# IllyaArtemchuk/Harmonies-Alphazero

Hardware: AMD Instinct MI355X
Metric: self-play env-steps/sec + games/sec @4096 boards, 1/2/4/8 GPUs; bit-exact vs CPU (higher is better)
Workload: dtype u64; 1 GPU; config2: 4096 concurrent boards/GPU, reset + rule-driven play to game end (legal mask, step, chance draws, final scoring); one step = 256 hz_play launches of 4096 boards; boards_per_gpu=4096, parallelism=shard1

## Files before the change

### harmonies-alphazero_amd/csrc/hz_env.hip

```cpp
#include <hip/hip_runtime.h>

#include <cstdio>
#include <cstdlib>
#include <cstring>

#include "../../include/hz_abi.h"
#include "hz_device.hpp"
#include "hz_encode.hpp"
#include "hz_host.hpp"

using namespace hz;
using namespace hz_host;

struct P2Draw {
  int32_t *tag;
  int32_t *k;
  uint64_t *q;
  uint64_t *bag;
  int32_t *c;
};
struct P2Mid {
  int32_t *tag;
  uint64_t *st;
  uint64_t *q;
  int32_t *i;
};

#ifndef HZ_P2_NDRAW
#define HZ_P2_NDRAW 6
#endif
#ifndef HZ_P2_NPLAY
#define HZ_P2_NPLAY 5
#endif
constexpr int kP2Draw = HZ_P2_NDRAW;
constexpr int kP2Play = HZ_P2_NPLAY;
constexpr int kP2SDraw = 4;
constexpr int kP2SPlay = kP2SDraw + kP2Draw;
constexpr int kP2Stages = kP2SPlay + kP2Play;
constexpr int kP2Last = kP2Stages - 1;
constexpr int kP2Ring = kP2Play + 1;
constexpr int kP2Stream = kP2Stages;
static_assert(kP2Draw >= 2 && kP2Draw <= 6 && kP2Play >= 2 && kP2Play <= 5, "stage counts");

struct hz_env {
  DevBufs bufs, p2_bufs, ar_bufs;
  int32_t n;
  uint64_t seed_base;
  hipStream_t stream;
  uint64_t *state;
  uint32_t *mt;
  int32_t *pos;
  int32_t *ply;
  int32_t *episode;
  uint64_t *seed;
  int seed_ahead;
  uint32_t *ahead_mt[2];
  int32_t *ahead_tag[2];
  uint64_t *ahead_pile[2];
  int32_t *ahead_cur[2];
  uint32_t *ahead_rule[2];
  int32_t *ep_final[2];
  size_t nrow;
  uint32_t *ring_mt[3];
  int32_t *ring_tag[3];
  uint64_t *ring_pile[3];
  int32_t *ring_cur[3];
  int32_t *ring_k1[3];
  int calls;
  int primed, slot_valid[2];
  int32_t *mt_src;
  int lazy;
  int ar_ahead;
  uint32_t *ar_mt;
  int32_t *ar_tag;
  uint64_t *ar_pile;
// ... 568 lines not shown
  a.seed_h[2] = e->p2_p3h[w];
  const int draws = e->seed_ahead;
  for (int k = 0; k < kP2Draw; k++) {
    P2DrawArgs &d = a.dr[k];
    const int s = kP2SDraw + k;
    d.slot = e->p2_s[sl(s)];
    d.stag = e->p2_s_tag[sl(s)];
    d.cur = e->p2_s_cur[sl(s)];
    d.in = e->p2_x[k > 0 ? k - 1 : 0][w];
    d.out = k == kP2Draw - 1 ? e->p2_pl[c % kP2Ring] : e->p2_x[k][r];
    d.d0 = e->p2_dcut[k];
    d.d1 = k == kP2Draw - 1 ? draws : std::min(draws, e->p2_dcut[k + 1]);
  }
  for (int st = 0; st < kP2Play; st++) {
    P2PlayArgs &p = a.pp[st];
    const bool last = st == kP2Play - 1;
    const int s = kP2SPlay + st;
    const int k = (c + kP2Ring - 1 - st) % kP2Ring;
    p.ep = last ? e->episode : e->p2_ep[w];
    p.ep_off = last ? 0 : kP2Play - 1 - st;
    p.g0 = st > 0 ? e->p2_cut[st - 1] : 0;
    p.g_end = last ? max_plies : std::min(e->p2_cut[st], max_plies);
    p.fell_lim = e->p2_fell_lim;
    p.ptag = e->p2_pl[k].tag;
    p.pk = e->p2_pl[k].k;
    p.q = st > 0 ? e->p2_m[st - 1][w].q : e->p2_pl[k].q;
    p.h = e->p2_h[sl(s)];
    p.slot = e->p2_s[sl(s)];
    p.cur = e->p2_s_cur[sl(s)];
    p.in = e->p2_m[st > 0 ? st - 1 : 0][w];
    p.out = e->p2_m[last ? 0 : st][r];
  }
  const int nblk = grid_for(e->n);
  hipLaunchKernelGGL(k_play2, dim3(4 * nblk), dim3(kStageThreads), kResetLds, e->stream, a, nblk);
  if (int err = launch_err()) return err;
  e->lazy = 1;
  e->calls2 = (c + 1) % (kP2Stream * kP2Ring * 2);
  e->primed = 0;
  e->ar_primed = 0;
  return 0;
}

extern "C" {

hz_env *hz_env_create(int32_t n_boards, uint64_t seed_base, void *stream) {
  if (n_boards <= 0) return nullptr;
  if (install_comp_table()) return nullptr;
  if (lds_opt_in<k_reset>(kResetLds) || lds_opt_in<k_rollout<false, false>>(kResetLds) ||
      lds_opt_in<k_rollout<false, true>>(kResetLds) || lds_opt_in<k_rollout<true, false>>(kResetLds) ||
      lds_opt_in<k_rollout<true, true>>(kResetLds) || lds_opt_in<k_play2>(kResetLds) ||
      lds_opt_in<k_mt_materialize2>(kResetLds))
    return nullptr;
  hz_env *e = new (std::nothrow) hz_env();
  if (!e) return nullptr;
  e->n = n_boards;
  e->seed_base = seed_base;
  e->stream = (hipStream_t)stream;
  const size_t n = (size_t)n_boards, nr = (n + kBlock - 1) / kBlock * kBlock, i32 = sizeof(int32_t);
  e->nrow = nr;
  DevBufs &o = e->bufs;
  o.get(e->state, n * 6 * sizeof(uint64_t), 0);
  o.get(e->mt, n * 624 * sizeof(uint32_t));
  o.get(e->pos, n * i32, 0);
  o.get(e->ply, n * i32, 0);
  o.get(e->episode, n * i32, 0);
  o.get(e->seed, n * sizeof(uint64_t), 0);
  o.get(e->mt_src, n * i32, 0xff);
// ... 325 lines not shown
  if (touch(e)) return 1;
  if (int err = materialize(e)) return err;
  hipLaunchKernelGGL(k_turn_op, dim3(grid_for(e->n)), dim3(kBlock), 0, e->stream, e->state, e->mt, e->pos, e->n, sel,
                     0);
  return launch_err();
}

int hz_end_turn(hz_env *e, const uint8_t *sel) {
  if (!e) return -1;
  if (touch(e)) return 1;
  if (int err = materialize(e)) return err;
  hipLaunchKernelGGL(k_turn_op, dim3(grid_for(e->n)), dim3(kBlock), 0, e->stream, e->state, e->mt, e->pos, e->n, sel,
                     1);
  return launch_err();
}

int hz_encode_states(const uint64_t *states, int64_t word_stride, int64_t item_stride, const int32_t *idx, int32_t m,
                     float *board, float *glob, void *stream) {
  if (!states || m < 0 || (!board && !glob)) return -1;
  if (m == 0) return 0;
  launch_encode(states, (long)word_stride, (long)item_stride, idx, m, board, glob, (hipStream_t)stream);
  return launch_err();
}

const char *hz_version(void) { return "hz 0.1 gfx950"; }

#ifdef HZ_DIAG
int hz_diag_set_stamps(uint64_t *p) {
  return hipMemcpyToSymbol(HIP_SYMBOL(g_stamps), &p, sizeof(p)) == hipSuccess ? 0 : 1;
}
int hz_diag_set_role_only(int r) {
  return hipMemcpyToSymbol(HIP_SYMBOL(g_role_only), &r, sizeof(r)) == hipSuccess ? 0 : 1;
}
#endif

}
```

### harmonies-alphazero_amd/csrc/hz_host.hpp

```cpp
#pragma once

#include <atomic>
#include <cstddef>
#include <cstdint>
#include <cstdio>
#include <cstdlib>
#include <new>
#include <vector>

namespace hz_host {

inline int env_int(const char *name, int dflt) {
  const char *e = getenv(name);
  return e ? atoi(e) : dflt;
}

inline int env_pick(const char *name, int special, int otherwise) {
  return env_int(name, otherwise) == special ? special : otherwise;
}

inline int env_clamped(const char *name, int dflt, int lo, int hi) {
  const int v = env_int(name, dflt);
  return v < lo ? lo : v > hi ? hi : v;
}
// ... 3 lines not shown
  int c[3];
  if (e && sscanf(e, "%d,%d,%d", &c[0], &c[1], &c[2]) == 3 && c[0] > 0 && c[1] > c[0] && c[2] > c[1] &&
      c[0] % 4 == 0 && c[1] % 4 == 0 && c[2] % 4 == 0)
    for (int k = 0; k < 3; k++) cut[k] = c[k];
}

inline bool env_cuts_n(const char *name, int *cut, int n, int step, int hi) {
  const char *e = getenv(name);
  if (!e || n < 1 || n > 8 || step < 1) return false;
  int c[8];
  for (int k = 0; k < n; k++) {
    if (*e < '0' || *e > '9') return false;
    long v = 0;
    for (; *e >= '0' && *e <= '9'; e++)
      if ((v = v * 10 + (*e - '0')) > hi) return false;
    if (v < step || v % step || (k && v <= c[k - 1])) return false;
    c[k] = (int)v;
    if (*e++ != (k + 1 < n ? ',' : '\0')) return false;
  }
  for (int k = 0; k < n; k++) cut[k] = c[k];
  return true;
}

inline bool cuts_gaps_within(const int *cut, int n, int max_gap) {
  for (int k = 0; k + 1 < n; k++)
    if (cut[k + 1] - cut[k] > max_gap) return false;
  return true;
}

inline bool env_p2_dcuts(const char *name, int *dcut, int ndraw, int draws, int max_gap) {
  if (ndraw < 2 || ndraw > 8) return false;
  int dc[9];
  for (int k = 0; k <= ndraw; k++) dc[k] = dcut[k];
  bool got = ndraw == 6 && env_cuts_n(name, dc + 1, 5, 1, draws);
  if (!got) {
    const int n = ndraw == 6 ? 4 : ndraw - 1;
    got = env_cuts_n(name, dc + 1, n, 1, draws - 1);
    if (got && ndraw == 6 && dc[5] < dc[4]) dc[5] = dc[4];
  }
  if (!got || !cuts_gaps_within(dc, ndraw + 1, max_gap)) return false;
  for (int k = 0; k <= ndraw; k++) dcut[k] = dc[k];
  return true;
}

struct Setting {
  static constexpr int64_t kUnread = INT64_MIN;
  const char *name;
  int32_t dflt;
  std::atomic<int64_t> v{kUnread};
  int32_t get() {
    int64_t x = v.load(std::memory_order_relaxed);
    if (x == kUnread) {
      int64_t expect = kUnread;
      v.compare_exchange_strong(expect, (int64_t)env_int(name, dflt));
      x = v.load(std::memory_order_relaxed);
    }
    return (int32_t)x;
  }
  void set(int32_t x) { v.store(x, std::memory_order_relaxed); }
};

template <class Dev>
struct DevBufsT {
  struct Held {
    void *p;
    void *slot;
    void (*clear)(void *slot);
  };
  std::vector<Held> held;
  bool ok = true;

// ... 71 lines not shown
```

### harmonies-alphazero_amd/csrc/hz_play2.hpp

```cpp
#pragma once

namespace {

#ifndef HZ_P2_ST_WT
#define HZ_P2_ST_WT 0
#endif
#ifndef HZ_P2_AUX
#define HZ_P2_AUX 16
#endif
#ifndef HZ_P2_STATIC_WIN
#define HZ_P2_STATIC_WIN 1
#endif
constexpr bool kP2StaticWin = HZ_P2_STATIC_WIN;

constexpr int kP2Win = 96;
constexpr int kP2WinRows = kP2Win + 24;
#ifndef HZ_P2_DCUT
#if HZ_P2_NDRAW == 6
#define HZ_P2_DCUT 0, 5, 9, 13, 17, 20
#elif HZ_P2_NDRAW == 5
#define HZ_P2_DCUT 0, 6, 11, 15, 19
#elif HZ_P2_NDRAW == 4
#define HZ_P2_DCUT 0, 7, 13, 18
#endif
#endif
constexpr int kP2DCut[kP2Draw] = {HZ_P2_DCUT};
constexpr int kP2StageDraws = 7;
#ifndef HZ_P2_PCUT
#if HZ_P2_NPLAY == 5
#define HZ_P2_PCUT 16, 32, 48, 64
#elif HZ_P2_NPLAY == 4
#define HZ_P2_PCUT 24, 40, 56
#endif
#endif
constexpr int kP2PCut[kP2Play - 1] = {HZ_P2_PCUT};
enum { kWvP1 = 8, kWvPlay = 10, kWvIdle = 15 };
#ifndef HZ_P2_WAVES
#if HZ_P2_NDRAW == 6 && HZ_P2_NPLAY == 5
#define HZ_P2_WAVES 0, 1, 4, 5, 2, 3, 8, 10
#elif HZ_P2_NDRAW == 6
#define HZ_P2_WAVES 0, 1, 4, 5, 2, 3, 8, 15
#elif HZ_P2_NDRAW == 5 && HZ_P2_NPLAY == 5
#define HZ_P2_WAVES 0, 1, 4, 15, 2, 3, 8, 10
#elif HZ_P2_NDRAW == 5
#define HZ_P2_WAVES 0, 1, 4, 15, 2, 3, 8, 15
#elif HZ_P2_NPLAY == 5
#define HZ_P2_WAVES 0, 1, 8, 15, 2, 3, 10, 15
#else
#define HZ_P2_WAVES 0, 1, 8, 15, 2, 3, 15, 15
#endif
#endif
constexpr int kP2Wave[8] = {HZ_P2_WAVES};
constexpr int p2_wave_count(int code) {
  int c = 0;
  for (int k = 0; k < 8; k++) c += kP2Wave[k] == code;
  return c;
}
constexpr bool p2_waves_ok() {
  for (int d = 0; d < 6; d++)
    if (p2_wave_count(d) != (d < kP2Draw ? 1 : 0)) return false;
  return p2_wave_count(kWvP1) == 1 && p2_wave_count(kWvPlay) == (kP2Play == 5 ? 1 : 0);
}
#ifndef HZ_P2_HSPLIT
#define HZ_P2_HSPLIT 24, 24, 52
#endif
constexpr int kP2HashSplit[3] = {HZ_P2_HSPLIT};
constexpr int kP2HashCut[5] = {0, kP2HashSplit[0], kP2HashSplit[1], kP2HashSplit[2], kRulePlies};
static_assert(0 <= kP2HashCut[1] && kP2HashCut[1] <= kP2HashCut[2] && kP2HashCut[2] <= kP2HashCut[3] &&
                  kP2HashCut[3] <= kRulePlies,
              "HZ_P2_HSPLIT: non-decreasing rows within the table");
static_assert(p2_waves_ok(), "HZ_P2_WAVES: every stage outside the seed and play blocks on exactly one wave");
constexpr int kP2MinPlies = 96;
#ifdef HZ_DIAG
constexpr int kP2Stamps = 48;
#define P2_PHASE(slot, t0)                                                                                       \
  do {                                                                                                           \
    __builtin_amdgcn_sched_barrier(0);                                                                           \
    if (g_stamps && b < a.n) g_stamps[(size_t)b * kP2Stamps + (slot)] = __builtin_amdgcn_s_memtime() - (t0); \
    __builtin_amdgcn_sched_barrier(0);                                                                           \
  } while (0)
#define P2_USE_V(x) asm volatile("" ::"v"(x))
#define P2_USE_S(x) asm volatile("" ::"s"(x))
#else
#define P2_PHASE(slot, t0) \
  do {                     \
  } while (0)
#define P2_USE_V(x) \
  do {              \
  } while (0)
#define P2_USE_S(x) \
  do {              \
  } while (0)
#endif
static_assert(4 * kP2WinRows * kWinStride * 4 <= (int)kResetLds, "a window per wave of a draw block");

struct P2DrawArgs {
  const uint32_t *slot;
  const int32_t *stag;
  int32_t *cur;
  P2Draw in, out;
  int d0, d1;
};
struct P2PlayArgs {
  const int32_t *ep;
  int ep_off;
  int g0;
  int g_end;
  int fell_lim;
  const int32_t *ptag, *pk;
  const uint64_t *q;
  const uint32_t *h;
  uint32_t *slot;
  const int32_t *cur;
  P2Mid in, out;
};
struct P2Args {
  uint64_t *st;
  uint32_t *mt;
  int32_t *pos, *ply, *episode;
  uint64_t *seed;
  int n, max_plies;
  uint64_t seed_base;
  long nrow;
  int32_t *games_done, *steps_done, *mt_src;
  int32_t *win_tag;
  const int32_t *ep_in;
  int32_t *ep_out;
  P2DrawArgs dr[kP2Draw];
  P2PlayArgs pp[kP2Play];
  uint32_t *s_mt[kP2SDraw];
  int32_t *s_tag[kP2SDraw];
  const int32_t *seed_tag[3];
  const uint32_t *seed_h[3];
  int s_idx_last;
  uint32_t *p1h_w;
  int32_t *p1t_w;
  uint32_t *p2h_w;
  uint32_t *p3h_w;
  uint32_t *s_h[kP2SDraw];
  int32_t *err;
  int spin;
};

struct PlayDraw2 : PileScript {
  bool fell;
  MTR gm;
  const int32_t *cur_nd;
  __device__ __forceinline__ bool pair_pops() const { return d + 2 <= nd; }
  __device__ __forceinline__ bool lost() const { return fell && gm.over(); }
  __device__ __forceinline__ uint32_t draw_one(uint64_t misc) {
    if (d < nd) return pop();
    if (!fell) {
      gm = MTR(gm.w, gm.stride, *cur_nd, gm.lim);
      fell = true;
    }
    uint32_t p9;
    return draw_pile(misc, gm, p9) ? p9 : 0x1FFu;
  }
  __device__ __forceinline__ uint32_t operator()(uint64_t misc) { return take(misc, true); }
  __device__ __forceinline__ uint32_t take(uint64_t misc, bool want) {
    if (__all(!want || d < nd)) return pop_if(want);
    return want ? draw_one(misc) : 0x1FFu;
  }
};

template <class Draw>
__device__ __forceinline__ int p2_plies(State &s, Draw &draw, int g, int g_end, uint64_t rkey, const uint32_t *hs,
                                        size_t nr, const uint32_t *h0 = nullptr, int h0_g = -1) {
  const int g0 = g;
  auto hash = [&](int ply) -> uint32_t { return hs && ply < kRulePlies ? hs[(size_t)ply * nr] : rule_h32(rkey, ply); };
  const bool all_hs = __all(hs != nullptr);
  uint32_t hn[8];
  int hn_g = -1;
  if (h0 && all_hs) {
#pragma unroll
// ... 64 lines not shown
  return *reinterpret_cast<const uint4 *>(p);
}
template <class T>
__device__ __forceinline__ T p2_at(const T *base, uint32_t off) {
  typedef __attribute__((address_space(1))) const char GlobalByte;
  typedef __attribute__((address_space(1))) const T GlobalT;
  return *(GlobalT *)((GlobalByte *)base + off);
}
template <class T>
__device__ __forceinline__ const T *p2_row(const T *base, size_t row_words) {
  const T *p = base + row_words;
  asm volatile("" : "+s"(p));
  return p;
}
__device__ __forceinline__ void p2_fence() { asm volatile("" ::: "memory"); }
__device__ __forceinline__ void p2_fence_use(int &x) { asm volatile("" : "+v"(x)::"memory"); }
template <class T>
__device__ __forceinline__ void p2_st(T *p, T v) {
  if constexpr (HZ_P2_AUX == 16 && HZ_P2_ST_WT) __hip_atomic_store(p, v, __ATOMIC_RELAXED, __HIP_MEMORY_SCOPE_AGENT);
  else *p = v;
}
__device__ __forceinline__ uint32_t p1_step(uint32_t t, uint32_t q, bool odd, uint32_t kA, uint32_t kB) {
  return (t ^ ((q ^ (q >> 30)) * 1664525U)) + (odd ? kA : kB);
}
__device__ __forceinline__ uint32_t p1_row1(uint32_t kA, uint32_t kB) {
  return p1_step(kInitGen.v[1], 19650218u, true, kA, kB);
}
__device__ __forceinline__ void p2_keys(uint64_t seed, uint32_t &kA, uint32_t &kB) {
  const uint32_t key0 = (uint32_t)seed, key1 = (uint32_t)(seed >> 32);
  kA = key0;
  kB = key1 ? key1 + 1u : key0;
}

template <int S>
__device__ __forceinline__ void p2_hash_rows(const P2Args &a, int b, uint64_t seed) {
  constexpr int J0 = kP2HashCut[S], J1 = kP2HashCut[S + 1];
  if constexpr (J0 < J1) {
    __builtin_amdgcn_sched_barrier(0);
    const size_t nr = (size_t)a.nrow;
    const uint64_t rk = rule_key(seed);
    uint32_t *h = a.s_h[S] + (size_t)J0 * nr + b;
#pragma unroll 1
    for (int j = J0; j < J1; j++, h += nr) p2_st(h, rule_h32(rk, j));
    __builtin_amdgcn_sched_barrier(0);
  }
}

typedef uint32_t u32x8 __attribute__((ext_vector_type(8)));
template <int Imm>
__device__ __forceinline__ u32x8 p1_load8(const uint32_t *tab, uint32_t off) {
  u32x8 t;
  asm volatile("s_load_dwordx8 %0, %1, %2 offset:%3" : "=&s"(t) : "s"(tab), "s"(off), "n"(Imm));
  return t;
}
__device__ __forceinline__ void p1_arrived(u32x8 &t) { asm volatile("s_waitcnt lgkmcnt(0)" : "+s"(t)); }
__device__ __forceinline__ uint32_t p1_steps8(const u32x8 &t, uint32_t prev, uint32_t kA, uint32_t kB) {
#pragma unroll
  for (int u = 0; u < 8; u++) prev = p1_step(t[u], prev, !(u & 1), kA, kB);
  return prev;
}
__device__ __forceinline__ void p2_p1(const P2Args &a, int b) {
  const int e = a.ep_in[b] + kP2Last;
  const uint64_t seed = episode_seed(a.seed_base, b, e);
  uint32_t kA, kB;
  p2_keys(seed, kA, kB);
  uint32_t prev = 19650218u;
  const uint32_t *tab = kInitGen.v + 1;
  static_assert(38 * 16 + 1 == 609 && 617 + 8 <= kMT + kInitGenPad, "the last group's read (rows 617-624) within the table's padding");
  u32x8 ta = p1_load8<0>(tab, 0), tb;
  p1_arrived(ta);
#pragma unroll 1
  for (uint32_t off = 0; off < 38 * 64; off += 64) {
    tb = p1_load8<32>(tab, off);
    __builtin_amdgcn_sched_barrier(0);
    prev = p1_steps8(ta, prev, kA, kB);
    __builtin_amdgcn_sched_barrier(0);
    p1_arrived(tb);
    ta = p1_load8<64>(tab, off);
    __builtin_amdgcn_sched_barrier(0);
    prev = p1_steps8(tb, prev, kA, kB);
    __builtin_amdgcn_sched_barrier(0);
    p1_arrived(ta);
  }
  tb = p1_load8<0>(tab, (617 - 1) * 4);
  prev = p1_steps8(ta, prev, kA, kB);
  p1_arrived(tb);
#pragma unroll
  for (int u = 0; u < 7; u++) prev = p1_step(tb[u], prev, !(u & 1), kA, kB);
  a.p1h_w[b] = p1_step(p1_row1(kA, kB), prev, false, kA, kB);
  p2_hash_rows<0>(a, b, seed);
  a.p1t_w[b] = e * 8 + 2;
}

#ifndef HZ_P2_BEND
#define HZ_P2_BEND 433
#endif
#ifndef HZ_P2_AEND
#define HZ_P2_AEND 209
#endif
#ifndef HZ_P2_LEAN
#define HZ_P2_LEAN 1
#endif
#ifndef HZ_P2_TWIST
#define HZ_P2_TWIST 160
#endif
constexpr int kP2Twist = HZ_P2_TWIST;
constexpr int kP2Ahead = 0 | (kP2Twist << 16);
static_assert(kP2Twist % 8 == 0 && kP2Twist >= 64 && kP2Twist <= kAheadTwist, "the slot's twisted rows");
constexpr int kP2PartEnd = HZ_P2_LEAN ? kP2Twist + 1 : kAheadTwist + 1;
constexpr int p2_up8(int from, int x) { return x <= from ? from : from + 8 * ((x - from + 7) / 8); }
constexpr int p2_min(int a, int b) { return a < b ? a : b; }
constexpr int kP2aEnd = HZ_P2_AEND, kP2bEnd = HZ_P2_BEND;
static_assert(kP2bEnd > 399 && kP2bEnd + 64 < kMT && (kP2bEnd - kAheadTwist - 1) % 8 == 0, "P2b's final steps in groups of eight; rows 397, 398 P2b's");
static_assert(kP2aEnd > 11 && kP2aEnd <= kAheadTwist - 7 && (kAheadTwist + 1 - kP2aEnd) % 8 == 0, "P2b's part steps in groups of eight");
constexpr int kP2bDrop = HZ_P2_LEAN ? kAheadTwist + 1 + 8 * ((397 - kAheadTwist - 1) / 8) : kAheadTwist + 1;
struct P2Ahead {
  uint32_t cur[8];
  uint32_t iv[8];
  uint32_t last;
};
typedef __attribute__((address_space(4))) const uint32_t ConstWord;
__device__ __forceinline__ ConstWord *p2_table() {
// ... 68 lines not shown
    }
    if (KeepLds) {
      p2_publish(prog, g + 8);
      lg += 8 * S * 4;
    }
    h.last = h.cur[7];
#pragma unroll
    for (int u = 0; u < 8; u++) {
      h.cur[u] = nx[u];
      h.iv[u] = ivn[u];
    }
  }
}
template <int G, int G1, int Mode>
__device__ __forceinline__ void p2_tail(const P2Out &o, int lane, uint32_t &prev, P2Ahead &h) {
  static_assert(G1 - G >= 1 && G1 - G <= 8, "within the group ahead");
  [[maybe_unused]] const int soff = __builtin_amdgcn_readfirstlane((Mode == kP2Part ? G - 1 : G) * o.row_bytes);
#pragma unroll
  for (int i = G; i < G1; i++) {
    const uint32_t v = (h.cur[i - G] ^ ((prev ^ (prev >> 30)) * 1566083941U)) - (uint32_t)i;
    if constexpr (p2_mode_hbm(Mode)) o.put(Mode == kP2Part ? twist_part(prev, v) : v, soff, i - G);
    if (p2_mode_lds(Mode)) hz_lds[i * kLdsStride + lane] = v;
    prev = v;
  }
  h.last = h.cur[G1 - G - 1];
}

template <int K>
__device__ __forceinline__ void p2_third(const P2Args &a, int b0, int lane, int e, bool ok, const uint32_t (&hw)[4],
                                         int *s_prog) {
  const int b = b0 + lane;
  const bool act = b < a.n;
  const size_t nr = (size_t)a.nrow;
  if (K == 0 && act && !ok) a.s_tag[1][b] = -1;
  if (!__any(ok)) {
    if (K == 2) p2_publish(s_prog, kMT + 1);
    return;
  }
  uint32_t *slot = a.s_mt[1 + K];
  const uint64_t seed = episode_seed(a.seed_base, b, e);
  uint32_t kA, kB;
  p2_keys(seed, kA, kB);
  uint32_t prev, first1, row2, q;
  if (K == 0) {
    first1 = act ? hw[0] : 0u;
    prev = first1;
    q = p1_row1(kA, kB);
  } else {
    prev = act ? hw[0] : 0u;
    first1 = act ? hw[1] : 0u;
    row2 = act ? hw[2] : 0u;
    q = act ? hw[3] : 0u;
  }
  const __amdgpu_buffer_rsrc_t rs = p2_slot_rsrc(slot, b0, nr);
  const int row_bytes = __builtin_amdgcn_readfirstlane((int)(nr * 4));
  const P2Out o(rs, row_bytes, lane);
  ConstWord *tab = p2_table();
  P2Ahead h;
  if constexpr (K == 0) {
    q = p1_step(kInitGen.v[2], q, false, kA, kB);
    row2 = (q ^ ((prev ^ (prev >> 30)) * 1566083941U)) - 2U;
    prev = row2;
    p2_ahead_init<3>(tab, h, q, kA, kB);
    constexpr int G = 3 + 8 * ((kP2aEnd - 3) / 8), Gp = p2_min(G, p2_up8(3, kP2PartEnd));
    p2_span<3, Gp, kP2Part>(tab, o, prev, h, kA, kB, s_prog);
    p2_span<Gp, G, kP2None>(tab, o, prev, h, kA, kB, s_prog);
    p2_tail<G, kP2aEnd, (G < kP2PartEnd ? kP2Part : kP2None)>(o, lane, prev, h);
  } else if constexpr (K == 1) {
    p2_ahead_init<kP2aEnd>(tab, h, q, kA, kB);
    constexpr int E1 = kAheadTwist + 1, Pb = p2_min(E1, p2_up8(kP2aEnd, kP2PartEnd));
    p2_span<kP2aEnd, Pb, kP2Part>(tab, o, prev, h, kA, kB, s_prog);
    p2_span<Pb, E1, kP2None>(tab, o, prev, h, kA, kB, s_prog);
    if constexpr (!HZ_P2_LEAN)
      __builtin_amdgcn_raw_buffer_store_b32(prev, rs, lane * 4, kAheadTwist * row_bytes, HZ_P2_AUX);
    p2_span<E1, kP2bDrop, kP2None>(tab, o, prev, h, kA, kB, s_prog);
    p2_span<kP2bDrop, kP2bEnd, kP2Final>(tab, o, prev, h, kA, kB, s_prog);
  } else {
    const uint32_t f0 = act ? slot[(size_t)397 * nr + b] : 0u, f1 = act ? slot[(size_t)398 * nr + b] : 0u;
// ... 4 lines not shown
    p2_span<kP2bEnd, Kc, Keep>(tab, o, prev, h, kA, kB, s_prog);
    p2_span<Kc, G, kP2None>(tab, o, prev, h, kA, kB, s_prog);
    p2_tail<G, kMT, (Kc == G ? Keep : kP2None)>(o, lane, prev, h);
    p2_publish(s_prog, kMT);
    const uint32_t row1 = (first1 ^ ((prev ^ (prev >> 30)) * 1566083941U)) - 1U;
    __builtin_amdgcn_raw_buffer_store_b32(f0 ^ twist_part(0x80000000u, row1), rs, lane * 4, 0, HZ_P2_AUX);
    __builtin_amdgcn_raw_buffer_store_b32(f1 ^ twist_part(row1, row2), rs, lane * 4, row_bytes, HZ_P2_AUX);
  }
  if (K < 2) {
    if (ok) {
      uint32_t *ho = K == 0 ? a.p2h_w : a.p3h_w;
      ho[b] = prev;
      ho[nr + b] = first1;
      ho[2 * nr + b] = row2;
      ho[3 * nr + b] = h.last;
      p2_hash_rows<1 + K>(a, b, seed);
      a.s_tag[1 + K][b] = e * 8 + 3 + K;
    }
  } else if (ok) {
    p2_hash_rows<3>(a, b, seed);
    a.s_tag[3][b] = e * 8 + 5;
  }
}

#ifndef HZ_P2_TWGO
#define HZ_P2_TWGO 64
#endif
constexpr int kTwGo = HZ_P2_TWGO;
constexpr int kTwIters = kP2Twist / 4;
constexpr int kTwHbm = (kP2bEnd - 397 + 3) / 4;
__device__ __forceinline__ uint4 xor4(const uint4 &a, const uint4 &b) {
  return make_uint4(a.x ^ b.x, a.y ^ b.y, a.z ^ b.z, a.w ^ b.w);
}
__device__ __forceinline__ void p2_twist(const P2Args &a, int b0, int lane, bool any, int *s_prog) {
  if (!any) return;
  const size_t nr = (size_t)a.nrow;
  uint32_t *slot = a.s_mt[3];
  const int grp = lane >> 4, c4 = (lane & 15) * 4;
  uint32_t *col = slot + b0 + c4;
  auto row = [&](int r) { return p2_ld4(col + (size_t)r * nr); };
  const __amdgpu_buffer_rsrc_t rs = p2_slot_rsrc(slot, b0, nr);
  const int row_bytes = __builtin_amdgcn_readfirstlane((int)(nr * 4));
  auto store = [&](int r, const uint4 &v) {
    typedef uint32_t v4u __attribute__((ext_vector_type(4)));
    __builtin_amdgcn_raw_buffer_store_b128(v4u{v.x, v.y, v.z, v.w}, rs, c4 * 4 + r * row_bytes, 0, HZ_P2_AUX);
  };
  [[maybe_unused]] const int b = b0 + lane;
  HZ_DIAG_T0(tz);
  int have = kTwGo >= 0 ? p2_wait(s_prog, kP2bEnd + kTwGo, a.spin, a.err) : 0;
  P2_PHASE(35, tz);
  uint4 pt[kTwIters], fh[kTwHbm];
#pragma unroll
  for (int i = 0; i < kTwIters; i++) {
    const int r = grp + 4 * i;
    pt[i] = r >= 2 ? row(r) : make_uint4(0, 0, 0, 0);
  }
#pragma unroll
  for (int i = 0; i < kTwHbm; i++) {
    const int r = grp + 4 * i + 397;
    fh[i] = r < kP2bEnd ? row(r) : make_uint4(0, 0, 0, 0);
  }
  auto far = [&](int i) -> uint4 {
    const int r = grp + 4 * i;
    if (i < kTwHbm && r + 397 < kP2bEnd) return fh[i < kTwHbm ? i : 0];
    const uint32_t *d = hz_lds + (r + 397) * kLdsStride + c4;
    return make_uint4(d[0], d[1], d[2], d[3]);
  };
#pragma unroll
  for (int i = 0; i < kTwIters; i += 2) {
    const int need = 4 * (i + 1) + 3 + 397 + 1;
    if (need > kP2bEnd && have < need) have = p2_wait(s_prog, need, a.spin, a.err);
    const uint4 f0 = far(i), f1 = far(i + 1);
    if (i > 0 || grp >= 2) store(grp + 4 * i, xor4(f0, pt[i]));
    store(grp + 4 * (i + 1), xor4(f1, pt[i + 1]));
    if (i == 0) P2_PHASE(36, tz);
  }
  P2_PHASE(37, tz);
}

__device__ __forceinline__ void p2_seed(const P2Args &a, int blk) {
  __shared__ int s_prog;
  const int tid = threadIdx.x, lane = tid & 63, w = tid >> 6;
  const int b0 = blk * kBlock, b = b0 + lane;
  const bool act = b < a.n;
  if (tid == 0) s_prog = 0;
  const int wv = __builtin_amdgcn_readfirstlane(w);
  const int k = wv < 3 ? wv : 2;
  const int32_t *tagp = a.seed_tag[k];
  const uint32_t *hp = a.seed_h[k];
  const int32_t *ep_in = a.ep_in;
  const int n = a.n;
  const size_t hrow = k == 0 ? 0 : (size_t)a.nrow;
  asm volatile("" ::"s"(tagp), "s"(hp), "s"(ep_in), "s"(n), "s"(hrow));
  __builtin_amdgcn_sched_barrier(0);
  const int bc = min(b, n - 1);
  const int hb = wv < 3 ? bc : b0;
  const uint32_t *hrp[4];
#pragma unroll
  for (int i = 0; i < 4; i++) hrp[i] = p2_row(hp, i * hrow);
  p2_fence();
  int ep = p2_at(ep_in, (uint32_t)bc * 4u);
  const int tag = p2_at(tagp, (uint32_t)bc * 4u);
  uint32_t hw[4];
#pragma unroll
  for (int i = 0; i < 4; i++) hw[i] = p2_at(hrp[i], (uint32_t)hb * 4u);
  p2_fence_use(ep);
  const int e = act ? ep + kP2Last - 1 - k : 0;
  const bool ok = act && tag == e * 8 + 2 + k;
  __syncthreads();
  if (w == 0) p2_third<0>(a, b0, lane, e, ok, hw, &s_prog);
  else if (w == 1) p2_third<1>(a, b0, lane, e, ok, hw, &s_prog);
  else if (w == 2) p2_third<2>(a, b0, lane, e, ok, hw, &s_prog);
  else p2_twist(a, b0, lane, __any(ok), &s_prog);
}

__device__ __forceinline__ P2DrawArgs p2_draw_args(const P2Args &a, int stage, int &n, size_t &nr,
                                                   const int32_t *&ep_in) {
  const P2DrawArgs r = a.dr[stage];
  n = a.n;
  nr = (size_t)a.nrow;
  ep_in = a.ep_in;
  asm volatile("" ::"s"(r.slot), "s"(r.stag), "s"(r.cur), "s"(r.in.tag), "s"(r.in.k), "s"(r.in.q), "s"(r.in.bag),
               "s"(r.in.c), "s"(r.out.tag), "s"(r.out.k), "s"(r.out.q), "s"(r.out.bag), "s"(r.out.c), "s"(r.d0),
               "s"(r.d1), "s"(n), "s"(nr), "s"(ep_in));
  __builtin_amdgcn_sched_barrier(0);
  return r;
}
__device__ __forceinline__ P2PlayArgs p2_play_args(const P2Args &a, int st, int &n, size_t &nr, uint64_t &seed_base) {
  const P2PlayArgs r = a.pp[st];
  n = a.n;
  nr = (size_t)a.nrow;
  seed_base = a.seed_base;
  asm volatile("" ::"s"(r.ep), "s"(r.ep_off), "s"(r.g0), "s"(r.g_end), "s"(r.ptag), "s"(r.pk), "s"(r.q), "s"(r.h),
               "s"(r.slot), "s"(r.cur), "s"(r.in.tag), "s"(r.in.st), "s"(r.in.q), "s"(r.in.i),
               "s"(r.out.tag), "s"(r.out.st), "s"(r.out.q), "s"(r.out.i), "s"(n), "s"(nr), "s"(seed_base),
               "s"(r.fell_lim));
  __builtin_amdgcn_sched_barrier(0);
  return r;
}
__device__ __forceinline__ int wave_min_i(int v) {
#pragma unroll
  for (int o = 32; o > 0; o >>= 1) v = min(v, __shfl_xor(v, o));
  return v;
}
__device__ __forceinline__ void p2_draw_stage(const P2Args &a, int b0, int lane, int stage, int base) {
  const int b = b0 + lane;
// ... 42 lines not shown
  p2_fence();
  if (kP2StaticWin || stage == 0) win_load(rs);
  p2_fence_use(ep);
  if (stage == 1) {
    P2_USE_V(ep);
    P2_PHASE(34, t0);
  }
  const int e = act ? ep + kP2Last - kP2SDraw - stage : 0;
  bool ok = act && stag == e * 8 + 5;
  if (stage > 0) {
    k0 = ik;
    c0 = ic;
    bag = ibag;
#pragma unroll
    for (int i = 0; i < kAheadWords; i++) q[i] = iq[i];
    ok = ok && itag == e * 8 + stage;
  }
  if (stage == 1) {
    P2_USE_V((int)ok);
    P2_PHASE(26, t0);
  }
  bool draws = ok && k0 >= d0 && d0 < d1;
  int r0 = rs;
  if constexpr (kP2StaticWin) {
    draws = draws && (c0 & 0xFFFF) >= r0;
    win_store();
  } else {
    r0 = wave_min_i(draws ? (c0 & 0xFFFF) : kP2Twist) & ~3;
    if (r0 < kP2Twist) {
      if (stage > 0) win_load(r0);
      win_store();
    }
  }
  P2_PHASE(stage < 5 ? 28 + stage : 43, t0);
  if (!act) return;
  if (!ok) {
    out.tag[b] = -1;
    return;
  }
  if (stage == 0) cur[0] = kP2Ahead;
  int k = k0, cc = c0;
  if (draws) {
    const int lim = min(r0 + kP2Win, kP2Twist);
    StreamDraw<WinMT> d{WinMT(base - r0 * kWinStride + lane, c0, lim)};
#pragma unroll 1
    for (int i = d0; i < d1; i++) {
      if (d.m.pos >= lim) break;
      const uint32_t p9 = d(bag);
      if (d.m.pos > lim) break;
      apply_pile_fast(bag, p9);
      const int bit = 9 * i, wd = bit >> 6, off = bit & 63;
      const uint64_t lo9 = (uint64_t)p9 << off, hi9 = off > 55 ? (uint64_t)p9 >> (64 - off) : 0ull;
      q[0] |= wd == 0 ? lo9 : 0ull;
      q[1] |= wd == 1 ? lo9 : wd == 0 ? hi9 : 0ull;
      q[2] |= wd == 2 ? lo9 : wd == 1 ? hi9 : 0ull;
      q[3] |= wd == 3 ? lo9 : wd == 2 ? hi9 : 0ull;
      cc = d.m.cursor();
      p2_st(&cur[(size_t)(i + 1) * nr], cc);
      k = i + 1;
    }
  }
  p2_st(&out.k[b], k);
  p2_st(&out.c[b], cc);
  p2_st(&out.bag[b], bag);
#pragma unroll
  for (int i = 0; i < kAheadWords; i++) p2_st(&out.q[(size_t)i * nr + b], q[i]);
  p2_st(&out.tag[b], e * 8 + stage + 1);
// ... 111 lines not shown
      P2_PHASE(17 + 2 * st, t0);
      if (draw.lost()) prep = false;
    }
    if (!last) {
      if (prep) p2_mid_put(mo, nr, b, s, draw, g, e);
      else mo.tag[b] = -1;
    } else {
      int cursor, src;
      if (prep) {
        cursor = draw.fell ? draw.gm.cursor() : cur[(size_t)draw.d * nr];
        src = 2 + a.s_idx_last;
      } else {
        mt_seed(hz_lds + lane, kLdsStride, sd);
        PlayDraw fb{{0, 0, 0, 0, 0, 0}, LdsMT(lane, kMTSeeded), false, false, MT(nullptr, 0), nullptr};
        reset_state(s, fb);
        g = p2_plies(s, fb, 0, a.max_plies, rk, nullptr, nr);
        cursor = fb.m.cursor();
        src = -1;
        lds_used = true;
      }
      a.episode[b] = e + 1;
      if (score_pending(s.misc)) finish_game(s);
      P2_PHASE(27, t0);
      store_state(a.st, a.n, b, s);
      a.pos[b] = cursor;
      a.mt_src[b] = src;
      a.win_tag[b] = -1;
      a.ply[b] = g;
      a.seed[b] = sd;
      a.ep_out[b] = e + 1;
      if (a.games_done) a.games_done[b] = phase_of(s.misc) == PH_OVER ? 1 : 0;
      if (a.steps_done) a.steps_done[b] = g;
    }
    if (in_block) P2_PHASE(w, t0);
  }
  if (!in_block) return;
  if (w == 0) {
    const uint64_t lm = __ballot(lds_used);
    if (lane == 0) s_lds_mask = lm;
  }
  __syncthreads();
  const uint64_t lds_mask = s_lds_mask & actmask;
  if (lds_mask) stage_mt(a.mt + (size_t)b0 * kMT, nb, tid, lds_mask, false);
}

__global__ void __launch_bounds__(kStageThreads) __attribute__((amdgpu_waves_per_eu(1, 1))) k_play2(P2Args a, int nblk) {
  const int blk = (int)blockIdx.x;
  const int role = blk / nblk;
  const int rb = blk - role * nblk;
  const int wv = __builtin_amdgcn_readfirstlane((int)(threadIdx.x >> 6));
  const int code = role == 1 || role == 2 ? kP2Wave[4 * (role - 1) + wv] : kWvIdle;
  const int st = role == 0 ? kP2Play - 1 - wv : code == kWvPlay ? 0 : -1;
#ifdef HZ_DIAG
  if (g_role_only >= 0 && g_role_only != role) return;
  const uint64_t t0 = __builtin_amdgcn_s_memtime(), r0 = __builtin_amdgcn_s_memrealtime();
#endif
  if (st >= 0) p2_play(a, rb, st, role == 0);
  else if (role == 3) p2_seed(a, rb);
  else if (role != 0) p2_draw(a, rb, code);
#ifdef HZ_DIAG
  {
    const int w = threadIdx.x >> 6, bb = rb * kBlock + (threadIdx.x & 63);
    const bool idle = (role == 1 || role == 2) && code == kWvIdle;
    if (g_stamps && role > 0 && !idle && bb < a.n) g_stamps[(size_t)bb * kP2Stamps + 4 * role + w] = __builtin_amdgcn_s_memtime() - t0;
    if (g_stamps && bb < a.n && (threadIdx.x & 63) < 4) {
      const int k = threadIdx.x & 63;
      const uint64_t v = k == 0 ? r0 : k == 1 ? __builtin_amdgcn_s_memrealtime() : k == 2 ? t0 : __builtin_amdgcn_s_memtime();
      g_stamps[(size_t)(rb * kBlock + 16 * role + 4 * w + k) * kP2Stamps + 40] = v;
      if (k == 0)
        g_stamps[(size_t)(rb * kBlock + 16 * role + 4 * w) * kP2Stamps + 41] =
            (uint64_t)__builtin_amdgcn_s_getreg((31 << 11) | 4) | ((uint64_t)__builtin_amdgcn_s_getreg((15 << 11) | 20) << 32);
    }
  }
#endif
}

__global__ void __launch_bounds__(kStageThreads) k_mt_materialize2(uint32_t *__restrict__ mt,
                                                                  const uint64_t *__restrict__ seed,
                                                                  const int32_t *__restrict__ pos,
                                                                  int32_t *__restrict__ mt_src, int n) {
  __shared__ uint64_t s_mask;
  const int tid = threadIdx.x, lane = tid & 63;
  const int b0 = blockIdx.x * kBlock, b = b0 + lane;
  const int nb = n - b0 < kBlock ? n - b0 : kBlock;
  if (tid < 64) {
    const int src = b < n ? mt_src[b] : -1;
    const bool mine = src >= 2 && src < 2 + kP2Stream;
    const uint64_t m = __ballot(mine);
    if (lane == 0) s_mask = m;
    if (mine) {
      mt_seed(hz_lds + lane, kLdsStride, seed[b]);
      LdsMT s(lane, kMTSeeded);
      s.twist_ahead(pos[b] >> 16);
      mt_src[b] = -1;
    }
  }
  __syncthreads();
  const uint64_t mask = s_mask;
  if (mask) stage_mt(mt + (size_t)b0 * kMT, nb, tid, mask, false);
}


}
// ... 1 lines not shown
```

Before: 25.88 billion env-steps/s.

## Widen k_play2 blocks to five waves, split draw into seven stages and twist in two

Makes k_play2 blocks five waves wide by default. The extra wave lets the draw pipeline use seven stages with finer cut points and a smaller window, and lets the seed block split the MT twist and rule-hash rows across two waves. The cold-path P1 word and hash rows move into the first third stage, and a per-role wave table replaces the old wave-code mapping. This aims to shorten the critical per-block stage latency by spreading work over more waves. The cost is more threads per block, an occupancy hint allowing two waves per EU, and more pipeline stages and state.

```diff
diff --git a/harmonies-alphazero_amd/csrc/hz_env.hip b/harmonies-alphazero_amd/csrc/hz_env.hip
--- a/harmonies-alphazero_amd/csrc/hz_env.hip
+++ b/harmonies-alphazero_amd/csrc/hz_env.hip
@@ -26,12 +26,21 @@
   int32_t *i;
 };
 
+#ifndef HZ_P2_BLOCK_WAVES
+#define HZ_P2_BLOCK_WAVES 5
+#endif
 #ifndef HZ_P2_NDRAW
+#if HZ_P2_BLOCK_WAVES >= 5
+#define HZ_P2_NDRAW 7
+#else
 #define HZ_P2_NDRAW 6
+#endif
 #endif
 #ifndef HZ_P2_NPLAY
 #define HZ_P2_NPLAY 5
 #endif
+constexpr int kP2BlockWaves = HZ_P2_BLOCK_WAVES;
+constexpr int kP2Threads = 64 * kP2BlockWaves;
 constexpr int kP2Draw = HZ_P2_NDRAW;
 constexpr int kP2Play = HZ_P2_NPLAY;
 constexpr int kP2SDraw = 4;
@@ -40,7 +49,9 @@
 constexpr int kP2Last = kP2Stages - 1;
 constexpr int kP2Ring = kP2Play + 1;
 constexpr int kP2Stream = kP2Stages;
-static_assert(kP2Draw >= 2 && kP2Draw <= 6 && kP2Play >= 2 && kP2Play <= 5, "stage counts");
+static_assert(kP2Draw >= 2 && kP2Draw <= 7 && kP2Play >= 2 && kP2Play <= 5, "stage counts");
+static_assert(kP2BlockWaves == 4 || kP2BlockWaves == 5, "k_play2's blocks: four waves, or five");
+static_assert(kP2Draw <= 7, "a draw tag is episode * 8 + stages done (1 .. kP2Draw): three bits");
 
 struct hz_env {
   DevBufs bufs, p2_bufs, ar_bufs;
@@ -675,7 +686,7 @@
     p.out = e->p2_m[last ? 0 : st][r];
   }
   const int nblk = grid_for(e->n);
-  hipLaunchKernelGGL(k_play2, dim3(4 * nblk), dim3(kStageThreads), kResetLds, e->stream, a, nblk);
+  hipLaunchKernelGGL(k_play2, dim3(4 * nblk), dim3(kP2Threads), kResetLds, e->stream, a, nblk);
   if (int err = launch_err()) return err;
   e->lazy = 1;
   e->calls2 = (c + 1) % (kP2Stream * kP2Ring * 2);
@@ -1067,6 +1078,7 @@
 int hz_diag_set_role_only(int r) {
   return hipMemcpyToSymbol(HIP_SYMBOL(g_role_only), &r, sizeof(r)) == hipSuccess ? 0 : 1;
 }
+int hz_diag_p2_block_waves(void) { return kP2BlockWaves; }
 #endif
 
 }
diff --git a/harmonies-alphazero_amd/csrc/hz_host.hpp b/harmonies-alphazero_amd/csrc/hz_host.hpp
--- a/harmonies-alphazero_amd/csrc/hz_host.hpp
+++ b/harmonies-alphazero_amd/csrc/hz_host.hpp
@@ -59,11 +59,12 @@
   if (ndraw < 2 || ndraw > 8) return false;
   int dc[9];
   for (int k = 0; k <= ndraw; k++) dc[k] = dcut[k];
-  bool got = ndraw == 6 && env_cuts_n(name, dc + 1, 5, 1, draws);
-  if (!got) {
-    const int n = ndraw == 6 ? 4 : ndraw - 1;
-    got = env_cuts_n(name, dc + 1, n, 1, draws - 1);
-    if (got && ndraw == 6 && dc[5] < dc[4]) dc[5] = dc[4];
+  const int shortest = ndraw >= 6 && ndraw <= 7 ? 4 : ndraw - 1;
+  bool got = false;
+  for (int n = ndraw - 1; n >= shortest && !got; n--) {
+    got = env_cuts_n(name, dc + 1, n, 1, n >= 5 ? draws : draws - 1);
+    for (int k = n + 1; got && k < ndraw; k++)
+      if (dc[k] < dc[n]) dc[k] = dc[n];
   }
   if (!got || !cuts_gaps_within(dc, ndraw + 1, max_gap)) return false;
   for (int k = 0; k <= ndraw; k++) dcut[k] = dc[k];
diff --git a/harmonies-alphazero_amd/csrc/hz_play2.hpp b/harmonies-alphazero_amd/csrc/hz_play2.hpp
--- a/harmonies-alphazero_amd/csrc/hz_play2.hpp
+++ b/harmonies-alphazero_amd/csrc/hz_play2.hpp
@@ -13,10 +13,12 @@
 #endif
 constexpr bool kP2StaticWin = HZ_P2_STATIC_WIN;
 
-constexpr int kP2Win = 96;
+constexpr int kP2Win = kP2BlockWaves >= 5 && kP2Draw >= 7 ? 80 : 96;
 constexpr int kP2WinRows = kP2Win + 24;
 #ifndef HZ_P2_DCUT
-#if HZ_P2_NDRAW == 6
+#if HZ_P2_NDRAW == 7
+#define HZ_P2_DCUT 0, 4, 8, 12, 15, 18, 21
+#elif HZ_P2_NDRAW == 6
 #define HZ_P2_DCUT 0, 5, 9, 13, 17, 20
 #elif HZ_P2_NDRAW == 5
 #define HZ_P2_DCUT 0, 6, 11, 15, 19
@@ -34,45 +36,76 @@
 #endif
 #endif
 constexpr int kP2PCut[kP2Play - 1] = {HZ_P2_PCUT};
-enum { kWvP1 = 8, kWvPlay = 10, kWvIdle = 15 };
-#ifndef HZ_P2_WAVES
-#if HZ_P2_NDRAW == 6 && HZ_P2_NPLAY == 5
-#define HZ_P2_WAVES 0, 1, 4, 5, 2, 3, 8, 10
-#elif HZ_P2_NDRAW == 6
-#define HZ_P2_WAVES 0, 1, 4, 5, 2, 3, 8, 15
-#elif HZ_P2_NDRAW == 5 && HZ_P2_NPLAY == 5
-#define HZ_P2_WAVES 0, 1, 4, 15, 2, 3, 8, 10
-#elif HZ_P2_NDRAW == 5
-#define HZ_P2_WAVES 0, 1, 4, 15, 2, 3, 8, 15
-#elif HZ_P2_NPLAY == 5
-#define HZ_P2_WAVES 0, 1, 8, 15, 2, 3, 10, 15
+#ifndef HZ_P2_TWIST2
+#define HZ_P2_TWIST2 (HZ_P2_BLOCK_WAVES >= 5)
+#endif
+constexpr bool kP2Twist2 = HZ_P2_TWIST2;
+static_assert(!kP2Twist2 || kP2BlockWaves >= 5, "the twist's second half runs on a seed block's fifth wave");
+enum { kWvP1 = 8, kWvIdle = 15, kWvPlay = 16, kWvSeed = 24 };
+#ifndef HZ_P2_ROLES
+#define P2_PLAY_WAVES kWvPlay + kP2Play - 1, kWvPlay + kP2Play - 2, kWvPlay + kP2Play - 3, kWvPlay + kP2Play - 4
+#define P2_SEED_WAVES kWvSeed, kWvSeed + 1, kWvSeed + 2, kWvSeed + 3
+#define P2_SEED_FIFTH (HZ_P2_TWIST2 ? kWvSeed + 4 : 15)
+#if HZ_P2_BLOCK_WAVES == 5 && HZ_P2_NDRAW == 7 && HZ_P2_NPLAY == 5
+#define HZ_P2_ROLES P2_PLAY_WAVES, 15, 0, 1, 4, 5, 6, 2, 3, 8, 16, 15, P2_SEED_WAVES, P2_SEED_FIFTH
+#elif HZ_P2_BLOCK_WAVES == 5 && HZ_P2_NDRAW == 6 && HZ_P2_NPLAY == 5
+#define HZ_P2_ROLES P2_PLAY_WAVES, 15, 0, 1, 4, 5, 15, 2, 3, 8, 16, 15, P2_SEED_WAVES, P2_SEED_FIFTH
+#elif HZ_P2_BLOCK_WAVES == 4 && HZ_P2_NDRAW == 6 && HZ_P2_NPLAY == 5
+#define HZ_P2_ROLES P2_PLAY_WAVES, 0, 1, 4, 5, 2, 3, 8, 16, P2_SEED_WAVES
+#elif HZ_P2_BLOCK_WAVES == 4 && HZ_P2_NDRAW == 6
+#define HZ_P2_ROLES P2_PLAY_WAVES, 0, 1, 4, 5, 2, 3, 8, 15, P2_SEED_WAVES
+#elif HZ_P2_BLOCK_WAVES == 4 && HZ_P2_NDRAW == 5 && HZ_P2_NPLAY == 5
+#define HZ_P2_ROLES P2_PLAY_WAVES, 0, 1, 4, 15, 2, 3, 8, 16, P2_SEED_WAVES
+#elif HZ_P2_BLOCK_WAVES == 4 && HZ_P2_NDRAW == 5
+#define HZ_P2_ROLES P2_PLAY_WAVES, 0, 1, 4, 15, 2, 3, 8, 15, P2_SEED_WAVES
+#elif HZ_P2_BLOCK_WAVES == 4 && HZ_P2_NDRAW == 4 && HZ_P2_NPLAY == 5
+#define HZ_P2_ROLES P2_PLAY_WAVES, 0, 1, 8, 15, 2, 3, 16, 15, P2_SEED_WAVES
+#elif HZ_P2_BLOCK_WAVES == 4 && HZ_P2_NDRAW == 4
+#define HZ_P2_ROLES P2_PLAY_WAVES, 0, 1, 8, 15, 2, 3, 15, 15, P2_SEED_WAVES
+#endif
+#endif
+constexpr int kP2Role[4][kP2BlockWaves] = {HZ_P2_ROLES};
+constexpr int p2_role_count(int code, int type_lo, int type_hi) {
+  int c = 0;
+  for (int t = type_lo; t <= type_hi; t++)
+    for (int k = 0; k < kP2BlockWaves; k++) c += kP2Role[t][k] == code;
+  return c;
+}
+constexpr bool p2_roles_ok() {
+  for (int d = 0; d < 8; d++)
+    if (p2_role_count(d, 1, 2) != (d < kP2Draw ? 1 : 0) || p2_role_count(d, 0, 3) != (d < kP2Draw ? 1 : 0)) return false;
+  if (p2_role_count(kWvP1, 1, 2) != 1 || p2_role_count(kWvP1, 0, 3) != 1) return false;
+  for (int st = 0; st < 8; st++) {
+    const int want = st < kP2Play ? 1 : 0;
+    if (p2_role_count(kWvPlay + st, 0, 2) != want || p2_role_count(kWvPlay + st, 3, 3) != 0) return false;
+  }
+  if (p2_role_count(kWvPlay + kP2Play - 1, 0, 0) != 1) return false;
+  for (int k = 0; k < kP2BlockWaves; k++)
+    if (kP2Role[3][k] != (k < 4 || kP2Twist2 ? kWvSeed + k : kWvIdle)) return false;
+  for (int t = 0; t < 4; t++)
+    for (int k = 0; k < kP2BlockWaves; k++) {
+      const int c = kP2Role[t][k];
+      if (c < 0 || c > kWvSeed + 4) return false;
+      if (t == 0 && c != kWvIdle && !(c >= kWvPlay && c < kWvPlay + kP2Play)) return false;
+    }
+  return true;
+}
+#ifndef HZ_P2_HSPLIT
+#if HZ_P2_TWIST2
+#define HZ_P2_HSPLIT 0, 0, 0
 #else
-#define HZ_P2_WAVES 0, 1, 8, 15, 2, 3, 15, 15
-#endif
-#endif
-constexpr int kP2Wave[8] = {HZ_P2_WAVES};
-constexpr int p2_wave_count(int code) {
-  int c = 0;
-  for (int k = 0; k < 8; k++) c += kP2Wave[k] == code;
-  return c;
-}
-constexpr bool p2_waves_ok() {
-  for (int d = 0; d < 6; d++)
-    if (p2_wave_count(d) != (d < kP2Draw ? 1 : 0)) return false;
-  return p2_wave_count(kWvP1) == 1 && p2_wave_count(kWvPlay) == (kP2Play == 5 ? 1 : 0);
-}
-#ifndef HZ_P2_HSPLIT
 #define HZ_P2_HSPLIT 24, 24, 52
 #endif
+#endif
 constexpr int kP2HashSplit[3] = {HZ_P2_HSPLIT};
-constexpr int kP2HashCut[5] = {0, kP2HashSplit[0], kP2HashSplit[1], kP2HashSplit[2], kRulePlies};
+constexpr int kP2HashCut[5] = {0, kP2HashSplit[0], kP2HashSplit[1], kP2HashSplit[2], kP2Twist2 ? kP2HashSplit[2] : kRulePlies};
 static_assert(0 <= kP2HashCut[1] && kP2HashCut[1] <= kP2HashCut[2] && kP2HashCut[2] <= kP2HashCut[3] &&
                   kP2HashCut[3] <= kRulePlies,
               "HZ_P2_HSPLIT: non-decreasing rows within the table");
-static_assert(p2_waves_ok(), "HZ_P2_WAVES: every stage outside the seed and play blocks on exactly one wave");
+static_assert(p2_roles_ok(), "HZ_P2_ROLES: every stage on exactly one wave, of a block type that can run it");
 constexpr int kP2MinPlies = 96;
 #ifdef HZ_DIAG
-constexpr int kP2Stamps = 48;
+constexpr int kP2Stamps = 56;
 #define P2_PHASE(slot, t0)                                                                                       \
   do {                                                                                                           \
     __builtin_amdgcn_sched_barrier(0);                                                                           \
@@ -92,7 +125,14 @@
   do {              \
   } while (0)
 #endif
-static_assert(4 * kP2WinRows * kWinStride * 4 <= (int)kResetLds, "a window per wave of a draw block");
+constexpr int p2_draw_waves() {
+  int hi = 0;
+  for (int t = 1; t <= 2; t++)
+    for (int k = 0; k < kP2BlockWaves; k++)
+      if (kP2Role[t][k] < kP2Draw && k + 1 > hi) hi = k + 1;
+  return hi;
+}
+static_assert(p2_draw_waves() * kP2WinRows * kWinStride * 4 <= (int)kResetLds, "a window per draw wave of a draw block");
 
 struct P2DrawArgs {
   const uint32_t *slot;
@@ -141,6 +181,7 @@
   int32_t *err;
   int spin;
 };
+static_assert(sizeof(P2Args) <= 4096, "k_play2's arguments within the 4 KB a kernel may take");
 
 struct PlayDraw2 : PileScript {
   bool fell;
@@ -271,14 +312,14 @@
   kB = key1 ? key1 + 1u : key0;
 }
 
-template <int S>
+template <int S, int Entry = S>
 __device__ __forceinline__ void p2_hash_rows(const P2Args &a, int b, uint64_t seed) {
   constexpr int J0 = kP2HashCut[S], J1 = kP2HashCut[S + 1];
   if constexpr (J0 < J1) {
     __builtin_amdgcn_sched_barrier(0);
     const size_t nr = (size_t)a.nrow;
     const uint64_t rk = rule_key(seed);
-    uint32_t *h = a.s_h[S] + (size_t)J0 * nr + b;
+    uint32_t *h = a.s_h[Entry] + (size_t)J0 * nr + b;
 #pragma unroll 1
     for (int j = J0; j < J1; j++, h += nr) p2_st(h, rule_h32(rk, j));
     __builtin_amdgcn_sched_barrier(0);
@@ -298,11 +339,7 @@
   for (int u = 0; u < 8; u++) prev = p1_step(t[u], prev, !(u & 1), kA, kB);
   return prev;
 }
-__device__ __forceinline__ void p2_p1(const P2Args &a, int b) {
-  const int e = a.ep_in[b] + kP2Last;
-  const uint64_t seed = episode_seed(a.seed_base, b, e);
-  uint32_t kA, kB;
-  p2_keys(seed, kA, kB);
+__device__ __forceinline__ uint32_t p2_p1_word(uint32_t kA, uint32_t kB) {
   uint32_t prev = 19650218u;
   const uint32_t *tab = kInitGen.v + 1;
   static_assert(38 * 16 + 1 == 609 && 617 + 8 <= kMT + kInitGenPad, "the last group's read (rows 617-624) within the table's padding");
@@ -326,7 +363,14 @@
   p1_arrived(tb);
 #pragma unroll
   for (int u = 0; u < 7; u++) prev = p1_step(tb[u], prev, !(u & 1), kA, kB);
-  a.p1h_w[b] = p1_step(p1_row1(kA, kB), prev, false, kA, kB);
+  return p1_step(p1_row1(kA, kB), prev, false, kA, kB);
+}
+__device__ __forceinline__ void p2_p1(const P2Args &a, int b) {
+  const int e = a.ep_in[b] + kP2Last;
+  const uint64_t seed = episode_seed(a.seed_base, b, e);
+  uint32_t kA, kB;
+  p2_keys(seed, kA, kB);
+  a.p1h_w[b] = p2_p1_word(kA, kB);
   p2_hash_rows<0>(a, b, seed);
   a.p1t_w[b] = e * 8 + 2;
 }
@@ -461,7 +505,8 @@
   const int b = b0 + lane;
   const bool act = b < a.n;
   const size_t nr = (size_t)a.nrow;
-  if (K == 0 && act && !ok) a.s_tag[1][b] = -1;
+  const bool cold = K == 0 && act && !ok;
+  if (K == 0) ok = act;
   if (!__any(ok)) {
     if (K == 2) p2_publish(s_prog, kMT + 1);
     return;
@@ -473,6 +518,13 @@
   uint32_t prev, first1, row2, q;
   if (K == 0) {
     first1 = act ? hw[0] : 0u;
+    if (__any(cold)) {
+      const uint32_t w1 = p2_p1_word(kA, kB);
+      if (cold) {
+        first1 = w1;
+        p2_hash_rows<0, 1>(a, b, seed);
+      }
+    }
     prev = first1;
     q = p1_row1(kA, kB);
   } else {
@@ -543,8 +595,11 @@
 __device__ __forceinline__ uint4 xor4(const uint4 &a, const uint4 &b) {
   return make_uint4(a.x ^ b.x, a.y ^ b.y, a.z ^ b.z, a.w ^ b.w);
 }
-__device__ __forceinline__ void p2_twist(const P2Args &a, int b0, int lane, bool any, int *s_prog) {
-  if (!any) return;
+template <int I0, int I1, int J0, int J1>
+__device__ __forceinline__ void p2_twist(const P2Args &a, int b0, int lane, int e, bool ok, int *s_prog) {
+  static_assert(I0 % 2 == 0 && I1 % 2 == 0 && 0 <= I0 && I0 < I1 && I1 <= kTwIters, "whole pairs of iterations");
+  static_assert(0 <= J0 && J0 <= J1 && J1 <= kRulePlies, "hash rows within the table");
+  if (!__any(ok)) return;
   const size_t nr = (size_t)a.nrow;
   uint32_t *slot = a.s_mt[3];
   const int grp = lane >> 4, c4 = (lane & 15) * 4;
@@ -559,34 +614,45 @@
   [[maybe_unused]] const int b = b0 + lane;
   HZ_DIAG_T0(tz);
   int have = kTwGo >= 0 ? p2_wait(s_prog, kP2bEnd + kTwGo, a.spin, a.err) : 0;
-  P2_PHASE(35, tz);
-  uint4 pt[kTwIters], fh[kTwHbm];
-#pragma unroll
-  for (int i = 0; i < kTwIters; i++) {
+  if constexpr (I0 == 0) P2_PHASE(35, tz);
+  constexpr int H1 = I1 < kTwHbm ? I1 : kTwHbm, NH = H1 > I0 ? H1 - I0 : 0;
+  uint4 pt[I1 - I0], fh[NH > 0 ? NH : 1];
+#pragma unroll
+  for (int i = I0; i < I1; i++) {
     const int r = grp + 4 * i;
-    pt[i] = r >= 2 ? row(r) : make_uint4(0, 0, 0, 0);
-  }
-#pragma unroll
-  for (int i = 0; i < kTwHbm; i++) {
+    pt[i - I0] = r >= 2 ? row(r) : make_uint4(0, 0, 0, 0);
+  }
+#pragma unroll
+  for (int i = I0; i < H1; i++) {
     const int r = grp + 4 * i + 397;
-    fh[i] = r < kP2bEnd ? row(r) : make_uint4(0, 0, 0, 0);
+    fh[i - I0] = r < kP2bEnd ? row(r) : make_uint4(0, 0, 0, 0);
+  }
+  __builtin_amdgcn_sched_barrier(0);
+  if constexpr (J0 < J1) {
+    if (ok) {
+      const uint64_t rk = rule_key(episode_seed(a.seed_base, b, e));
+      uint32_t *h = a.s_h[3] + (size_t)J0 * nr + b;
+#pragma unroll 1
+      for (int j = J0; j < J1; j++, h += nr) p2_st(h, rule_h32(rk, j));
+    }
+    __builtin_amdgcn_sched_barrier(0);
   }
   auto far = [&](int i) -> uint4 {
     const int r = grp + 4 * i;
-    if (i < kTwHbm && r + 397 < kP2bEnd) return fh[i < kTwHbm ? i : 0];
+    if (i < H1 && r + 397 < kP2bEnd) return fh[i < H1 ? i - I0 : 0];
     const uint32_t *d = hz_lds + (r + 397) * kLdsStride + c4;
     return make_uint4(d[0], d[1], d[2], d[3]);
   };
 #pragma unroll
-  for (int i = 0; i < kTwIters; i += 2) {
+  for (int i = I0; i < I1; i += 2) {
     const int need = 4 * (i + 1) + 3 + 397 + 1;
     if (need > kP2bEnd && have < need) have = p2_wait(s_prog, need, a.spin, a.err);
     const uint4 f0 = far(i), f1 = far(i + 1);
-    if (i > 0 || grp >= 2) store(grp + 4 * i, xor4(f0, pt[i]));
-    store(grp + 4 * (i + 1), xor4(f1, pt[i + 1]));
-    if (i == 0) P2_PHASE(36, tz);
-  }
-  P2_PHASE(37, tz);
+    if (i > 0 || grp >= 2) store(grp + 4 * i, xor4(f0, pt[i - I0]));
+    store(grp + 4 * (i + 1), xor4(f1, pt[i + 1 - I0]));
+    if (I0 == 0 && i == 0) P2_PHASE(36, tz);
+  }
+  if constexpr (I0 == 0) P2_PHASE(37, tz);
 }
 
 __device__ __forceinline__ void p2_seed(const P2Args &a, int blk) {
@@ -622,7 +688,11 @@
   if (w == 0) p2_third<0>(a, b0, lane, e, ok, hw, &s_prog);
   else if (w == 1) p2_third<1>(a, b0, lane, e, ok, hw, &s_prog);
   else if (w == 2) p2_third<2>(a, b0, lane, e, ok, hw, &s_prog);
-  else p2_twist(a, b0, lane, __any(ok), &s_prog);
+  else if constexpr (kP2Twist2) {
+    constexpr int Ih = kTwIters / 2 & ~1, Jh = kRulePlies / 2;
+    if (w == 3) p2_twist<0, Ih, 0, Jh>(a, b0, lane, e, ok, &s_prog);
+    else p2_twist<Ih, kTwIters, Jh, kRulePlies>(a, b0, lane, e, ok, &s_prog);
+  } else if (w == 3) p2_twist<0, kTwIters, 0, 0>(a, b0, lane, e, ok, &s_prog);
 }
 
 __device__ __forceinline__ P2DrawArgs p2_draw_args(const P2Args &a, int stage, int &n, size_t &nr,
@@ -731,7 +801,7 @@
       win_store();
     }
   }
-  P2_PHASE(stage < 5 ? 28 + stage : 43, t0);
+  P2_PHASE(stage < 5 ? 28 + stage : stage == 5 ? 43 : 53, t0);
   if (!act) return;
   if (!ok) {
     out.tag[b] = -1;
@@ -909,43 +979,48 @@
       if (a.games_done) a.games_done[b] = phase_of(s.misc) == PH_OVER ? 1 : 0;
       if (a.steps_done) a.steps_done[b] = g;
     }
-    if (in_block) P2_PHASE(w, t0);
+    if (in_block && w < 4) P2_PHASE(w, t0);
   }
   if (!in_block) return;
-  if (w == 0) {
+  if (last) {
     const uint64_t lm = __ballot(lds_used);
     if (lane == 0) s_lds_mask = lm;
   }
   __syncthreads();
   const uint64_t lds_mask = s_lds_mask & actmask;
-  if (lds_mask) stage_mt(a.mt + (size_t)b0 * kMT, nb, tid, lds_mask, false);
-}
-
-__global__ void __launch_bounds__(kStageThreads) __attribute__((amdgpu_waves_per_eu(1, 1))) k_play2(P2Args a, int nblk) {
+  if (lds_mask && tid < kStageThreads) stage_mt(a.mt + (size_t)b0 * kMT, nb, tid, lds_mask, false);
+}
+
+__global__ void __launch_bounds__(kP2Threads) __attribute__((amdgpu_waves_per_eu(1, kP2BlockWaves > 4 ? 2 : 1)))
+k_play2(P2Args a, int nblk) {
   const int blk = (int)blockIdx.x;
   const int role = blk / nblk;
   const int rb = blk - role * nblk;
   const int wv = __builtin_amdgcn_readfirstlane((int)(threadIdx.x >> 6));
-  const int code = role == 1 || role == 2 ? kP2Wave[4 * (role - 1) + wv] : kWvIdle;
-  const int st = role == 0 ? kP2Play - 1 - wv : code == kWvPlay ? 0 : -1;
+  const int code = kP2Role[role][wv];
+  const int st = code >= kWvPlay && code < kWvPlay + kP2Play ? code - kWvPlay : -1;
 #ifdef HZ_DIAG
   if (g_role_only >= 0 && g_role_only != role) return;
   const uint64_t t0 = __builtin_amdgcn_s_memtime(), r0 = __builtin_amdgcn_s_memrealtime();
 #endif
   if (st >= 0) p2_play(a, rb, st, role == 0);
+  else if (role == 0) __syncthreads();
   else if (role == 3) p2_seed(a, rb);
-  else if (role != 0) p2_draw(a, rb, code);
+  else p2_draw(a, rb, code);
 #ifdef HZ_DIAG
   {
     const int w = threadIdx.x >> 6, bb = rb * kBlock + (threadIdx.x & 63);
-    const bool idle = (role == 1 || role == 2) && code == kWvIdle;
-    if (g_stamps && role > 0 && !idle && bb < a.n) g_stamps[(size_t)bb * kP2Stamps + 4 * role + w] = __builtin_amdgcn_s_memtime() - t0;
+    const bool idle = code == kWvIdle;
+    if (g_stamps && role > 0 && !idle && bb < a.n)
+      g_stamps[(size_t)bb * kP2Stamps + (w < 4 ? 4 * role + w : 48 + role)] = __builtin_amdgcn_s_memtime() - t0;
     if (g_stamps && bb < a.n && (threadIdx.x & 63) < 4) {
-      const int k = threadIdx.x & 63;
+      const int k = threadIdx.x & 63, so = role < 2 ? 0 : 4;
+      const int col = 4 * (kP2BlockWaves * (role & 1) + w);
+      if (rb * kBlock + col + 3 >= a.n) return;
       const uint64_t v = k == 0 ? r0 : k == 1 ? __builtin_amdgcn_s_memrealtime() : k == 2 ? t0 : __builtin_amdgcn_s_memtime();
-      g_stamps[(size_t)(rb * kBlock + 16 * role + 4 * w + k) * kP2Stamps + 40] = v;
+      g_stamps[(size_t)(rb * kBlock + col + k) * kP2Stamps + 40 + so] = v;
       if (k == 0)
-        g_stamps[(size_t)(rb * kBlock + 16 * role + 4 * w) * kP2Stamps + 41] =
+        g_stamps[(size_t)(rb * kBlock + col) * kP2Stamps + 41 + so] =
             (uint64_t)__builtin_amdgcn_s_getreg((31 << 11) | 4) | ((uint64_t)__builtin_amdgcn_s_getreg((15 << 11) | 20) << 32);
     }
   }
```

Result: slower. 23.26 billion env-steps/s (-10.1%).
